# tvlearn/evo

Measured on AMD Instinct MI355X. Metric: E-step candidate-state evals/sec (NxS), full EM iteration, higher is better.
Workload: dtype f64; 1 GPU; ES3C D=256 H=512 S=200 N=100k f64 (north-star shape); algo=es3c, N_total=100000, N_rank0=100000, D=256, H=512, S=200, step=10 full EM iterations, world_size_rccl=1, ea=fit/randflip 10 parents x 1 child x 1 gen, states=p_init_Kn=1/H (init_states default), rng=device, mstep=device, parallelism=dp1

## Files before the change

### evo_amd/csrc/evo_amd.hip

```cpp
#include "../../include/evo_amd.h"

#include <dlfcn.h>
#include <math.h>
#include <stdarg.h>
#include <stdio.h>
#include <stdlib.h>
#include <string.h>

#include <atomic>
#include <chrono>
#include <memory>
#include <string>
#include <type_traits>
#include <vector>

#include "common.hpp"
#include "gemm_f64.hpp"
#include "kernels_bsc.hpp"
#include "kernels_common.hpp"
#include "kernels_evolve.hpp"
#include "kernels_mstep.hpp"
#include "kernels_sssc.hpp"
#include "kernels_sssc_quad.hpp"
#include "kernels_fused.hpp"
// ... 1906 lines not shown
  double expect = lv.scale * c->res_cnt[src] * ((tag == 0) ? 1.0 : 1.0 + (double)c->Cmax / (double)c->S);
  if (tag != 0 && level == 0) expect = (double)total;
  unsigned want = (unsigned)(2.0 * expect / per_block) + 4;
  return want < g ? want : g;
}

static bool use_k8_kernel(const evoamd_ctx *c, const LevelHints &lv) {
  const int tag = lv.known_tag;
  if (c->k8_mode >= 0) return c->k8_mode != 0;
  if (!c->need_known || tag == 2) return true;
  const double expect = c->res_cnt[tag == 0 ? 1 : 0] * (tag == 0 ? 1.0 : (double)c->Cmax / (double)c->S) +
                        (tag == 0 ? 0.0 : c->res_cnt[1]);
  return expect > 8192.0;
}

static bool few_dense_states(const evoamd_ctx *c, const LevelHints &lv) {
  const int tag = lv.known_tag;
  if (!c->need_known || tag == 2) return false;
  const double expect = lv.scale * (tag == 0 ? c->res_cnt[1] : c->res_cnt[1] + c->res_cnt[0] * (double)c->Cmax / (double)c->S);
  return expect <= 1024.0;
}

static bool few_above4(const evoamd_ctx *c, const LevelHints &lv) {
  if (!c->merge_small || !c->need_known || lv.known_tag == 2) return false;
  const double expect = lv.scale * c->res_cnt[1] * (1.0 + 4.0 * (double)c->Cmax / (double)std::max(1, c->S));
  return expect <= 256.0;
}

static int zero_lists(evoamd_ctx *c) {
  if (!c->lists_clean) {
    if (c->pending_skip)
      check_lists_kernel<<<1, 256, 0, c->stream>>>(c->list_n, 4 * LIST_SHARDS, c->pending_skip, c->err);
    else
      HIP_TRY(hipMemsetAsync(c->list_n, 0, 4 * LIST_SHARDS * sizeof(int), c->stream));
  }
  on_lists_claimed(c);
  return 0;
}

static int skip_mask(const bool need[3]) { return (need[0] ? 0 : 1) | (need[1] ? 0 : 2) | (need[2] ? 0 : 4); }

static bool census_mode(const evoamd_ctx *c) {
  return c->model == EVOAMD_MODEL_SSSC && c->clist && c->clist_n && c->ovf_rec && c->use_digest && c->dig && !c->mask_infr;
}

static int ensure_census(evoamd_ctx *c) {
  if (c->census_gen == c->kn_gen) return 0;
  const i64 total = c->N * (i64)c->S;
  if (!c->clist_clean) check_lists_kernel<<<1, 256, 0, c->stream>>>(c->clist_n, 4 * LIST_SHARDS, c->census_skip, c->err);
  on_census_claimed(c);
  unsigned grid = cdiv(total, CENSUS_T * CENSUS_PPT);
  if (grid > (unsigned)(8 * c->n_cu)) grid = (unsigned)(8 * c->n_cu);
  SpanGuard g(c, KID_MISC);
  census_kernel<<<grid, CENSUS_T, 0, c->stream>>>(c->dig, total, c->clist, (i64)c->clist_words(), c->clist_n, (int)list_cap(total), c->err);
  HIP_TRY(hipGetLastError());
  DBG_SYNC(c, "census");
  if (c->debug_poison_list) {
    c->debug_poison_list = 0;
    const int bad[1] = {0x7FFFFFF0}, one[1] = {1};
    HIP_TRY(hipMemcpyAsync(c->clist, bad, sizeof(int), hipMemcpyHostToDevice, c->stream));
    HIP_TRY(hipMemcpyAsync(c->clist_n, one, sizeof(int), hipMemcpyHostToDevice, c->stream));
    HIP_TRY(hipStreamSynchronize(c->stream));
    on_census_poisoned(c);
    return 0;
  }
  made_census(c);
  return 0;
}

static unsigned quad_grid(const evoamd_ctx *c, const LevelHints &lv, int level, i64 total, unsigned cap) {
  return level_grid(c, lv, level, total * 4, cap, 64);
}

static unsigned pb_clamp(const PairBins &pb, unsigned grid) {
  return pb.ent && grid > (unsigned)pb.nwg ? (unsigned)pb.nwg : grid;
}
#define PB_GRID_CHECK(pb, grid) \
  REQUIRE(!(pb).ent || (i64)(grid) <= (i64)(pb).nwg, "pair bins: producer grid exceeds the regions per bin (pb.nwg)")

template <class F>
static void with_hw(int hw, F &&f) {
  switch (hw) {
    case 1: f(std::integral_constant<int, 1>{}); break;
    case 2: f(std::integral_constant<int, 2>{}); break;
    case 4: f(std::integral_constant<int, 4>{}); break;
    case 8: f(std::integral_constant<int, 8>{}); break;
    case 16: f(std::integral_constant<int, 16>{}); break;
    default: f(std::integral_constant<int, 0>{}); break;
  }
}

template <typename F>
static void with_spl(int S, F &&f) {
  if (S <= 64) f(std::integral_constant<int, 1>{});
  else if (S <= 128) f(std::integral_constant<int, 2>{});
  else if (S <= 256) f(std::integral_constant<int, 4>{});
  else if (S <= 512) f(std::integral_constant<int, 8>{});
  else f(std::integral_constant<int, 16>{});
}
template <typename F>
static void with_cpl(int Cmax, F &&f) {
  if (Cmax <= 64) f(std::integral_constant<int, 1>{});
  else f(std::integral_constant<int, 4>{});
}

struct Es3cLists {
  ListOut o1, o2, o3;
  ListIn i1, i2, i3;
  ListIn cA, cB, cC;
  ListIn empty;
  ListOut none_out;
  ListIn none_in;
};

static Es3cLists es3c_lists(const evoamd_ctx *c, int cap) {
  Es3cLists ls = {};
  ls.o1 = {c->list1, c->list_n + 0 * LIST_SHARDS, cap};
  ls.o2 = {c->list2, c->list_n + 1 * LIST_SHARDS, cap};
  ls.o3 = {c->list3, c->list_n + 2 * LIST_SHARDS, cap};
  ls.i1 = {ls.o1.items, ls.o1.counts, cap};
  ls.i2 = {ls.o2.items, ls.o2.counts, cap};
  ls.i3 = {ls.o3.items, ls.o3.counts, cap};
  if (c->clist && c->clist_n) {
    ls.cA = {c->clist, c->clist_n, cap};
    ls.cB = {c->clist + c->clist_words(), c->clist_n + LIST_SHARDS, cap};
    ls.cC = {c->clist + 2 * c->clist_words(), c->clist_n + 2 * LIST_SHARDS, cap};
    ls.empty = {c->clist, c->clist_n + 3 * LIST_SHARDS, 0};
  }
  return ls;
}

template <int MODE, int TAG>
static int census_wavefront_levels(evoamd_ctx *c, const SsscArgs &a, const Es3cLists &ls, const bool need[3], bool few4,
                                   const LevelHints &lv, i64 total) {
  if (few4) {
    sssc_big_kernel<MODE, TAG><<<std::max(64u, level_grid(c, lv, 1, total * 256, 1024, 1)), 64, big_lds(SSSC_KCAP), c->stream>>>(
        a, need[1] ? ls.cB : ls.empty, ls.none_out, SSSC_KCAP, need[2] ? ls.cC : ls.empty, ls.i3);
    return 4;
  }
  sssc_big_kernel<MODE, TAG><<<std::max(256u, level_grid(c, lv, 2, total * 256, 8192, 1)), 64, big_lds(16), c->stream>>>(
      a, need[2] ? ls.cC : ls.empty, ls.o2, 16, ls.i3);
  if (!need[2]) return 4;
  sssc_big_kernel<MODE, TAG><<<level_grid(c, lv, 2, total * 256, 1024, 1), 64, big_lds(SSSC_KCAP), c->stream>>>(
      a, ls.i2, ls.none_out, SSSC_KCAP);
  return 2 | 4;
}

#define MAIN_LPJ_LDS_MAX (48 * 1024)

static size_t main_lpj_lds(int C, int H) {
  return ((size_t)(1024 / C + 2) * H + (H <= 512 ? (size_t)4 * H : 0)) * sizeof(double);
}

enum LpjRoute {
  LPJ_MASKED,
  LPJ_CENSUS,
  LPJ_CHAINS,
  LPJ_ROUND2
};
enum LpjMain {
  LPJ_MAIN_NONE,
  LPJ_MAIN_CENSUS,
  LPJ_MAIN_STAGED,
  LPJ_MAIN_UNSTAGED,
  LPJ_MAIN_SMALL
};

struct LpjPlan {
  LpjRoute route;
  LevelHints lv;
  int kid_main;
  i64 total;
  int cap;
  Es3cLists ls;
  bool need[3];
  bool any;
  LpjMain main;
  int rows_cap, stage_dg;
  size_t lds;
  unsigned grid;
  bool few4;
  bool k8;
  bool few_dense;
};

static void lpj_plan(const evoamd_ctx *c, const SsscArgs &a, int tag, const LevelHints &lv, int kid_main, LpjPlan &p) {
  p = LpjPlan{};
  p.lv = lv;
  p.kid_main = kid_main;
  p.total = a.N * (i64)a.C;
  p.cap = (int)list_cap(p.total);
  p.ls = es3c_lists(c, p.cap);
  levels_for(c, lv, p.need);
  p.any = p.need[0] || p.need[1] || p.need[2];
  const bool tables = !a.shared && (a.H % 2) == 0;
  const bool staged = tables && main_lpj_lds(a.C, a.H) <= MAIN_LPJ_LDS_MAX;
  if (a.mask)
    p.route = LPJ_MASKED;
  else if (tag == 0 && a.states == c->states && census_mode(c) && staged)
    p.route = LPJ_CENSUS;
  else
    p.route = c->census_opt ? LPJ_CHAINS : LPJ_ROUND2;
  p.stage_dg = a.H <= 512;
  p.grid = cdiv(p.total, 1024);
  if (staged) {
    p.main = p.route == LPJ_CENSUS ? (lv.levels_only ? LPJ_MAIN_NONE : LPJ_MAIN_CENSUS) : LPJ_MAIN_STAGED;
    p.rows_cap = 1024 / a.C + 2;
    p.lds = main_lpj_lds(a.C, a.H);
  } else if (tables && a.dig && c->main_unstaged) {
    p.main = LPJ_MAIN_UNSTAGED;
    p.lds = (p.stage_dg ? (size_t)4 * a.H : 0) * sizeof(double);
  } else {
    p.main = LPJ_MAIN_SMALL;
    p.grid = cdiv(p.total, 512);
  }
  p.few4 = p.route != LPJ_ROUND2 && few_above4(c, lv);
  p.k8 = p.route == LPJ_ROUND2 && use_k8_kernel(c, lv);
  p.few_dense = p.route == LPJ_ROUND2 && few_dense_states(c, lv);
}

static int lpj_sssc_masked(evoamd_ctx *c, const SsscArgs &a, const LpjPlan &p) {
  SpanGuard g(c, p.kid_main);
  const int gridm = (int)std::min<i64>(p.total, 65536);
  sssc_big_kernel<0><<<gridm, 64, big_lds(8), c->stream>>>(a, p.ls.none_in, p.ls.o3, 8);
  sssc_big_kernel<0><<<1024, 64, big_lds(SSSC_KCAP), c->stream>>>(a, p.ls.i3, p.ls.none_out, SSSC_KCAP);
  HIP_TRY(hipGetLastError());
  return 0;
}

template <int TAG>
static int lpj_sssc_main(evoamd_ctx *c, const SsscArgs &a, const LpjPlan &p) {
  if (p.main == LPJ_MAIN_NONE) return 0;
  SpanGuard g(c, p.kid_main);
  if (p.main == LPJ_MAIN_SMALL)
    sssc_small_kernel<2, 0, TAG, 512><<<p.grid, 512, 0, c->stream>>>(a, p.ls.none_in, p.ls.o1, PairBins{});
  else
    with_hw(a.HW, [&](auto hw) {
      constexpr int HWT = decltype(hw)::value;
      if (p.main == LPJ_MAIN_CENSUS)
        sssc_main_lpj_kernel<TAG, 512, HWT, 2, false><<<p.grid, 512, p.lds, c->stream>>>(a, p.ls.none_out, p.rows_cap, p.stage_dg);
      else if (p.main == LPJ_MAIN_STAGED)
        sssc_main_lpj_kernel<TAG, 512, HWT, 2><<<p.grid, 512, p.lds, c->stream>>>(a, p.ls.o1, p.rows_cap, p.stage_dg);
      else
        sssc_main_lpj_kernel<TAG, 512, HWT, 2, true, false><<<p.grid, 512, p.lds, c->stream>>>(a, p.ls.o1, 0, p.stage_dg);
    });
  HIP_TRY(hipGetLastError());
  DBG_SYNC(c, p.main == LPJ_MAIN_CENSUS ? "sssc lpj main (census)" : "sssc lpj main");
  return 0;
}

template <int TAG>
static int lpj_sssc_census_levels(evoamd_ctx *c, const SsscArgs &a, const LpjPlan &p, int &served) {
  const Es3cLists &ls = p.ls;
  SpanGuard g(c, KID_LPJ_OVF);
  if (p.need[0]) {
    SpanGuard gl(c, KID_LPJ_K34);
    sssc_quad_kernel<1, 0, TAG><<<quad_grid(c, p.lv, 0, p.total, 2048), 256, 0, c->stream>>>(a, ls.cA, ls.none_out, ls.o3, PairBins{}, nullptr);
  }
  DBG_SYNC(c, "sssc lpj quad level 3..4");
  if (p.need[1] && !p.few4) {
    SpanGuard gl(c, KID_LPJ_K58);
    sssc_quad_kernel<2, 0, TAG><<<quad_grid(c, p.lv, 1, p.total, 2048), 256, 0, c->stream>>>(a, ls.cB, ls.none_out, ls.o3, PairBins{}, nullptr);
  }
  DBG_SYNC(c, "sssc lpj quad level 5..8");
  SpanGuard gl(c, KID_LPJ_K9P);
  served = census_wavefront_levels<0, TAG>(c, a, ls, p.need, p.few4, p.lv, p.total);
  HIP_TRY(hipGetLastError());
  DBG_SYNC(c, p.few4 ? "sssc lpj census levels (merged)" : "sssc lpj census levels");
  return 0;
}

template <int TAG>
static int lpj_sssc_chain_levels(evoamd_ctx *c, const SsscArgs &a, const LpjPlan &p, int &served) {
  const Es3cLists &ls = p.ls;
  SpanGuard g(c, KID_LPJ_OVF);
  if (p.need[0])
    sssc_quad_kernel<1, 0, TAG><<<quad_grid(c, p.lv, 0, p.total, 2048), 256, 0, c->stream>>>(a, ls.i1, ls.o2, ls.o3, PairBins{}, nullptr);
  DBG_SYNC(c, "sssc lpj chain 3..4");
  if (p.few4) {
    sssc_big_kernel<0, TAG><<<std::max(64u, level_grid(c, p.lv, 1, p.total * 256, 1024, 1)), 64, big_lds(SSSC_KCAP), c->stream>>>(
        a, ls.i2, ls.none_out, SSSC_KCAP, ls.i3);
    served = 2 | 4;
  } else {
    if (p.need[1])
      sssc_quad_kernel<2, 0, TAG><<<quad_grid(c, p.lv, 1, p.total, 2048), 256, 0, c->stream>>>(a, ls.i2, ls.o3, ls.o3, PairBins{}, nullptr);
    DBG_SYNC(c, "sssc lpj chain 5..8");
    sssc_big_kernel<0, TAG><<<level_grid(c, p.lv, 2, p.total * 256, 1024, 1), 64, big_lds(SSSC_KCAP), c->stream>>>(
        a, ls.i3, ls.none_out, SSSC_KCAP);
    served = 4;
  }
  HIP_TRY(hipGetLastError());
  DBG_SYNC(c, p.few4 ? "sssc lpj chain wavefront level (merged)" : "sssc lpj chain wavefront level");
  return 0;
}

template <int TAG>
static int lpj_sssc_round2_levels(evoamd_ctx *c, const SsscArgs &a, const LpjPlan &p, int &served) {
  const Es3cLists &ls = p.ls;
  SpanGuard g(c, KID_LPJ_OVF);
  if (p.need[0])
    sssc_small_kernel<4, 0, TAG, 256><<<level_grid(c, p.lv, 0, p.total, 1024, 256), 256, 0, c->stream>>>(a, ls.i1, ls.o2, PairBins{}, ls.o3);
  DBG_SYNC(c, "sssc lpj K=4 level");
  bool merged23 = false;
  if (p.k8) {
    if (p.need[1])
      sssc_small_kernel<8, 0, TAG, 256><<<level_grid(c, p.lv, 1, p.total, 256, 256), 256, 0, c->stream>>>(a, ls.i2, ls.o3, PairBins{}, ls.o3);
  } else if (p.need[1] && p.few_dense) {
    sssc_big_kernel<0, TAG><<<level_grid(c, p.lv, 1, p.total * 256, 1024, 1), 64, big_lds(SSSC_KCAP), c->stream>>>(
        a, ls.i2, ls.none_out, SSSC_KCAP, ls.i3);
    merged23 = true;
  } else if (p.need[1]) {
    sssc_big_kernel<0, TAG><<<level_grid(c, p.lv, 1, p.total * 256, 4096, 1), 64, big_lds(8), c->stream>>>(a, ls.i2, ls.o3, 8);
  }
  DBG_SYNC(c, "sssc lpj K=8 level");
  if ((p.need[2] || c->sing_screen) && !merged23)
    sssc_big_kernel<0, TAG><<<level_grid(c, p.lv, 2, p.total * 256, 1024, 1), 64, big_lds(SSSC_KCAP), c->stream>>>(
        a, ls.i3, ls.none_out, SSSC_KCAP);
  served = (merged23 || p.need[2] || c->sing_screen) ? 4 : 0;
  HIP_TRY(hipGetLastError());
  DBG_SYNC(c, "sssc lpj wavefront level");
  return 0;
}

template <int TAG>
static int launch_sssc_lpj(evoamd_ctx *c, const SsscArgs &a, int kid_main, const LevelHints &lv) {
  TRY(zero_lists(c));
  LpjPlan p;
  lpj_plan(c, a, TAG, lv, kid_main, p);
  if (p.route == LPJ_MASKED) return lpj_sssc_masked(c, a, p);
  if (p.route == LPJ_CENSUS) TRY(ensure_census(c));
  TRY(lpj_sssc_main<TAG>(c, a, p));
  int served = 0;
  if (p.any)
    TRY(p.route == LPJ_CENSUS   ? lpj_sssc_census_levels<TAG>(c, a, p, served)
        : p.route == LPJ_CHAINS ? lpj_sssc_chain_levels<TAG>(c, a, p, served)
                                : lpj_sssc_round2_levels<TAG>(c, a, p, served));
  on_levels_skipped(c, p.route == LPJ_CENSUS, skip_mask(p.need), served, p.any);
  return 0;
}

static int launch_lpj(evoamd_ctx *c, const Batch &b, const LevelHints &lv) {
  if (c->model == EVOAMD_MODEL_BSC) return launch_bsc_lpj(c, b);
  SsscArgs a = sssc_args(c, b);
  if (b.tag == 0) return launch_sssc_lpj<0>(c, a, b.kid, lv);
  if (b.tag == 1) return launch_sssc_lpj<1>(c, a, b.kid, lv);
  return launch_sssc_lpj<2>(c, a, b.kid, lv);
}

static int check_err(evoamd_ctx *c) {
  int *e = c->h_err;
  HIP_TRY(hipMemcpyAsync(e, c->err, 4 * sizeof(int), hipMemcpyDeviceToHost, c->stream));
  HIP_TRY(hipStreamSynchronize(c->stream));
  if (e[0]) {
    HIP_TRY(hipMemsetAsync(c->err, 0, sizeof(int), c->stream));
    if (e[0] & 4) return fail(EVOAMD_E_INVALID, "internal: an ES3C overflow level was skipped although its list was not empty");
    if (e[0] & EVO_ERR_LIST_FULL) return fail(EVOAMD_E_INVALID, "internal: an ES3C overflow list was full, states were dropped");
    if (e[0] & EVO_ERR_BAD_ENTRY) return fail(EVOAMD_E_INVALID, "internal: an ES3C list entry or latent index read back from LDS was out of range");
    if (e[0] & 1) return fail(EVOAMD_E_KLIMIT, "ES3C: a state has more than %d active latents", SSSC_KCAP);
    return fail(EVOAMD_E_SINGULAR, "ES3C: exactly singular k x k system (the reference takes pinv here)");
  }
  return 0;
}

static int lpj_resident_launch(evoamd_ctx *c, double *out, const LevelHints &lv) {
  TRY(ensure_B(c));
  on_lpj_overwritten(c);
  if (c->S_perm) {
    allzero_lpj_kernel<<<cdiv(c->N, 256), 256, 0, c->stream>>>(c->yy, c->N, c->dpar, c->model == EVOAMD_MODEL_SSSC,
                                                               out, c->L, c->flags + 2 * c->N, c->err);
    HIP_TRY(hipGetLastError());
  }
  Batch b = {c->states, nullptr, c->Y, c->Bm, c->yy, c->N, c->S, 0, out, c->L, c->S_perm, c->flags, KID_LPJ_RES, 0};
  b.mask = c->mask_infr;
  SpanGuard pass(c, KID_LPJ_PASS);
  return launch_lpj(c, b, lv);
}

static int estep_resident_pass(evoamd_ctx *c) {
  if (c->prefetch_gen == c->gen) {
    drop_prefetch(c);
    std::swap(c->lpj, c->lpj_alt);
    return 0;
  }
  return lpj_resident_launch(c, c->lpj, batch_hints(c, 0));
}

static int estep_check_ready(const evoamd_ctx *c) {
  REQUIRE(c && c->configured && c->have_data && c->have_params, "configure, upload_data and set_params first");
  return 0;
}
static int estep_check_parents(const evoamd_ctx *c, int n_parents) {
  REQUIRE(n_parents >= 1 && n_parents <= c->S && n_parents <= 64, "n_parents must be in [1, min(S, 64)]");
  return 0;
}
static int estep_check_randflip(const evoamd_ctx *c, int n_parents, int n_children) {
  TRY(estep_check_ready(c));
  TRY(estep_check_parents(c, n_parents));
  REQUIRE(n_children >= 1 && n_children <= EV_MAX_CHILDREN && n_children <= c->H, "n_children must be in [1, min(8, H)]");
  REQUIRE(n_parents * n_children <= c->Cmax, "n_parents * n_children exceeds the configured Cmax");
  return 0;
// ... 2733 lines not shown
```

### evo_amd/csrc/kernels_sssc.hpp

```cpp
#pragma once
#include "common.hpp"
#include "kernels_mstep.hpp"
#include "pair_bins.hpp"

struct __attribute__((aligned(64))) PairEntry {
  double g01;
  double L;
  double l00, l01, l10, l11;
  double pad[2];
};
__device__ __forceinline__ bool pair_singular_L(double L) { return L == __builtin_inf(); }
__device__ __forceinline__ bool pair_singular_lam(double l00) { return !(fabs(l00) <= 1.7976931348623157e308); }

struct __attribute__((aligned(16))) OvfRec {
  unsigned short idx[8];
  double qn;
  double pad;
  double z[8];
};
static_assert(sizeof(OvfRec) == 96, "OvfRec is six 16-byte loads");

#define CS_SLICES 16
struct SsscArgs {
  const u64 *states;
// ... 593 lines not shown
      base = __shfl(base, leader, 64);
      if (over[p]) buf[base + __popcll(mask & ((1ull << lane) - 1ull))] = value[p];
    }
  }
  lds_barrier();
  if (threadIdx.x == 0) {
    const int n = ctl[0];
    ctl[1] = n ? atomicAdd(&lo.counts[shard], n) : 0;
  }
}
template <int BS>
__device__ __forceinline__ void append_begin(const ListOut &lo, int shard, int value, bool over, int *buf, int *ctl) {
  const int v[1] = {value};
  const bool o[1] = {over};
  append_begin<BS, 1>(lo, shard, v, o, buf, ctl);
}
template <int BS>
__device__ __forceinline__ void append_end(const ListOut &lo, int shard, const int *buf, const int *ctl, int *err = nullptr) {
  lds_barrier();
  const int n = ctl[0], start = ctl[1];
  if (n == 0) return;
  if (start < 0 || start + n > lo.cap) {
    if (err && threadIdx.x == 0) atomicOr(err, EVO_ERR_LIST_FULL);
    return;
  }
  const i64 dst = (i64)shard * lo.cap + start;
  for (int i = threadIdx.x; i < n; i += BS) lo.items[dst + i] = buf[i];
}

__device__ __forceinline__ double sssc_k2_value(const int k, const int idx0, const int idx1, const double4 *D1t, const double *Bn,
                                                const PairEntry &pe, const double yyn, const double s, int *err) {
#pragma clang fp contract(off)
  double4 d0 = make_double4(0.0, 0.0, 0.0, 0.0), d1 = make_double4(0.0, 0.0, 0.0, 0.0);
  double b0 = 0.0, b1 = 0.0, g01 = 0.0, L = 0.0, l00 = 0.0, l01 = 0.0, l10 = 0.0, l11 = 0.0;
  if (k >= 1) {
    d0 = D1t[idx0];
    b0 = Bn[idx0];
    L = d0.y;
    l00 = d0.w;
  }
  if (k == 2) {
    d1 = D1t[idx1];
    b1 = Bn[idx1];
    g01 = pe.g01;
    L = pe.L;
    l00 = pe.l00;
    l01 = pe.l01;
    l10 = pe.l10;
    l11 = pe.l11;
    if (pair_singular_L(pe.L) && pair_singular_lam(pe.l00)) atomicOr(err, 2);
  }
  const double v0 = fma(-g01, d1.x, fma(-d0.z, d0.x, b0));
  const double v1 = fma(-d1.z, d1.x, fma(-g01, d0.x, b1));
  const double rr = fma(-d1.x, b1 + v1, fma(-d0.x, b0 + v0, yyn));
  const double t0 = fma(l01, v1, l00 * v0), t1 = fma(l11, v1, l10 * v0);
  const double quad = fma(v1, t1, v0 * t0);
  return fma(-0.5 * s, fma(-s, quad, rr), L);
}

template <int TAG, int BS, int HWT, int PPT, bool APPEND = true, bool STAGEB = true>
__global__ __launch_bounds__(BS) void sssc_main_lpj_kernel(SsscArgs a, ListOut lo, int rows_cap, int stage_dg) {
  a.s2inv = a.dpar[DP_S2INV];
  extern __shared__ double smem[];
  __shared__ int ovf_buf[BS * PPT];
  __shared__ int ovf_ctl[2];
  double *Bs = smem;
  double4 *DGs = (double4 *)(smem + (STAGEB ? (size_t)rows_cap * a.H : 0));
  const i64 total = a.N * (i64)a.C;
  const i64 t0 = (i64)blockIdx.x * (BS * PPT);
  const i64 n_first = t0 / a.C;
  i64 n_last = (t0 + BS * PPT - 1) / a.C;
  if (n_last > a.N - 1) n_last = a.N - 1;
  const int rows = (int)(n_last - n_first + 1);
  bool live[PPT], over[PPT];
  int nloc[PPT], c[PPT], ktot[PPT], idx0[PPT], idx1[PPT], tv[PPT];
  double yyn[PPT];
  const float rC = 1.0f / (float)a.C;
#pragma unroll
  for (int p = 0; p < PPT; p++) {
    const i64 t = t0 + threadIdx.x + (i64)p * BS;
    tv[p] = (int)t;
    live[p] = t < total;
    nloc[p] = c[p] = ktot[p] = idx0[p] = idx1[p] = 0;
    yyn[p] = 0.0;
    if (live[p]) {
      const int off = (int)(t - n_first * a.C);
      int r = (int)(((float)off + 0.5f) * rC);
      if (r * a.C > off) r--;
      if ((r + 1) * a.C <= off) r++;
      nloc[p] = r;
      c[p] = off - r * a.C;
      live[p] = !(a.counts && c[p] >= a.counts[n_first + r]);
    }
  }
  u64 dgv[PPT];
#pragma unroll
  for (int p = 0; p < PPT; p++) {
    dgv[p] = 0ull;
    if (a.dig) {
      const i64 tc = live[p] ? (n_first + nloc[p]) * (i64)a.C + c[p] : 0;
      dgv[p] = a.dig[tc];
    } else if (live[p]) {
      const i64 n = n_first + nloc[p];
      load_state_k2<HWT>(a.states + ((a.shared ? 0 : n * (i64)a.C) + c[p]) * a.HW, a.HW, ktot[p], idx0[p], idx1[p]);
    }
    yyn[p] = a.yy[live[p] ? n_first + nloc[p] : 0];
  }
  {
    if (STAGEB) {
      const double2 *src = (const double2 *)(a.Bm + n_first * a.H);
      double2 *dst = (double2 *)Bs;
      const int n2 = rows * a.H / 2;
      for (int i = threadIdx.x; i < n2; i += BS) dst[i] = src[i];
    }
    if (stage_dg)
      for (int i = threadIdx.x; i < a.H; i += BS) DGs[i] = a.D1[i];
  }
  PairEntry pe[PPT];
#pragma unroll
  for (int p = 0; p < PPT; p++) {
    if (a.dig && live[p]) {
      ktot[p] = dig_k(dgv[p]);
      idx0[p] = dig_idx(dgv[p], 0);
      idx1[p] = dig_idx(dgv[p], 1);
    }
    over[p] = live[p] && ktot[p] > 2;
    const bool pair = live[p] && ktot[p] == 2;
    pe[p] = a.PT[pair ? (i64)idx0[p] * a.H + idx1[p] : 0];
  }
  const int shard = (int)(blockIdx.x & (LIST_SHARDS - 1));
  if (APPEND)
    append_begin<BS, PPT>(lo, shard, tv, over, ovf_buf, ovf_ctl);
  else
    lds_barrier();
  const double4 *D1t = stage_dg ? DGs : a.D1;
  const double s = a.s2inv;
#pragma unroll
  for (int p = 0; p < PPT; p++) {
    if (live[p] && !over[p]) {
      const int k = ktot[p];
      const double *Bn = STAGEB ? Bs + (size_t)nloc[p] * a.H
                                : a.Bm + (n_first + nloc[p]) * (i64)a.H;
      const double val = sssc_k2_value(k, idx0[p], idx1[p], D1t, Bn, pe[p], yyn[p], s, a.err);
      unsigned fl = 0;
      const i64 n = n_first + nloc[p];
      a.lpj_out[n * a.ldo + a.col0 + c[p]] = clamp_lpj(val, fl);
      if (fl) {
        atomicOr(&a.flags[n], fl);
        atomicOr(&a.err[1], 1);
      }
    }
  }
  if (APPEND) append_end<BS>(lo, shard, ovf_buf, ovf_ctl, a.err);
}

template <int HWT, int W, bool CEN = false>
__global__ __launch_bounds__(64 * W, W == 4 ? 2 : 1) void sssc_stats_wave_kernel(SsscArgs a, ListOut lo, PairBins pb, int stage,
                                                                                const OvfRec *__restrict__ rec = nullptr,
                                                                                const int rec_kmax = 8) {
  a.s2inv = a.dpar[DP_S2INV];
  extern __shared__ double wrows[];
  __shared__ int bcnt[PB_MAX_BINS];
  constexpr int OVB = 64;
  __shared__ int obuf[W][2 * OVB];
  const int H = a.H, lane = lane_id(), wave = wave_id_uniform();
  double *rowS = wrows + (size_t)wave * 2 * H, *rowZ = rowS + H;
  double *accS = wrows + (size_t)W * 2 * H, *accZ = accS + H, *accD = accZ + H;
  double *rowB = accD + H + (size_t)wave * H;
  double4 *d1s = (double4 *)(accD + H + (size_t)W * H);
  const bool binned = pb.ent != nullptr;
  for (int i = threadIdx.x; i < 3 * H; i += 64 * W) accS[i] = 0.0;
  if (HWT > 0 || stage)
    for (int i = threadIdx.x; i < H; i += 64 * W) d1s[i] = a.D1[i];
  if (binned)
    for (int i = threadIdx.x; i < pb.nb; i += 64 * W) bcnt[i] = CEN ? pb.gcnt[(size_t)i * pb.nwg + blockIdx.x] : 0;
  __syncthreads();
  const int shard = (int)(blockIdx.x & (LIST_SHARDS - 1));
  const double s = a.s2inv;
  int ocnt = 0;
  auto flush_obuf = [&]() {
    int base = 0;
    if (lane == 0) base = atomicAdd(&lo.counts[shard], ocnt);
    base = __shfl(base, 0, 64);
    for (int i = lane; i < ocnt; i += 64) {
      const int pos = base + i;
      if (pos >= 0 && pos < lo.cap)
        lo.items[(i64)shard * lo.cap + pos] = obuf[wave][i];
      else
        atomicOr(a.err, EVO_ERR_LIST_FULL);
    }
    ocnt = 0;
    lds_wave_fence();
  };
  constexpr bool PF = HWT > 0;
  constexpr int HB = PF ? HWT : 1;
  struct Pre {
    double rmax, rsum, B[HB], l[4];
    u64 d[4];
  };
  auto issue = [&](i64 nn, Pre &p) {
    p.rmax = a.rowmax[nn];
    p.rsum = a.rowsum[nn];
    const double *Bnn = a.Bm + nn * H;
#pragma unroll
    for (int i = 0; i < HB; i++) {
      const int h = lane + 64 * i;
      p.B[i] = Bnn[h < H ? h : H - 1];
    }
    const double *lpn = a.lpj_in + nn * a.ldo + a.col0;
    const u64 *dgn = a.dig + nn * (i64)a.C;
#pragma unroll
    for (int u = 0; u < 4; u++) {
      const int c = 64 * u + lane, cc = c < a.C ? c : 0;
      p.d[u] = dgn[cc];
      p.l[u] = lpn[cc];
    }
  };
  const i64 n_first = (i64)blockIdx.x * W + wave, n_stride = (i64)gridDim.x * W;
  Pre cur = {};
  if (PF && n_first < a.N) issue(n_first, cur);
  for (i64 n = n_first; n < a.N; n += n_stride) {
    const i64 n_next = n + n_stride < a.N ? n + n_stride : n;
    for (int h = lane; h < 2 * H; h += 64) rowS[h] = 0.0;
    double rmax, rsum;
    const double *Bn = a.Bm + n * H;
    if (PF) {
      rmax = cur.rmax;
      rsum = cur.rsum + EVO_F64_TINY;
#pragma unroll
      for (int i = 0; i < HB; i++) {
        const int h = lane + 64 * i;
        if (h < H) rowB[h] = cur.B[i];
      }
      Bn = rowB;
    } else {
      rmax = a.rowmax[n];
      rsum = a.rowsum[n] + EVO_F64_TINY;
      if (stage) {
        for (int h = lane; h < H; h += 64) rowB[h] = Bn[h];
        Bn = rowB;
      }
    }
    const double4 *D1t = (PF || stage) ? d1s : a.D1;
    const double *lp = a.lpj_in + n * a.ldo + a.col0;
    lds_wave_fence();
    auto group = [&](const int c0, auto first_tag) {
      constexpr bool first = decltype(first_tag)::value;
      constexpr int RG = 4;
      bool live[RG];
      int k[RG], idx0[RG], idx1[RG];
      double l[RG];
#pragma unroll
      for (int u = 0; u < RG; u++) {
        const int c = c0 + 64 * u + lane;
        live[u] = c < a.C;
        k[u] = idx0[u] = idx1[u] = 0;
        l[u] = 0.0;
        if (first) {
          const u64 d = cur.d[u];
          k[u] = live[u] ? dig_k(d) : 0;
          idx0[u] = dig_idx(d, 0);
          idx1[u] = dig_idx(d, 1);
          l[u] = cur.l[u];
        } else {
          if (a.dig) {
            const u64 d = a.dig[n * (i64)a.C + (live[u] ? c : 0)];
            k[u] = live[u] ? dig_k(d) : 0;
            idx0[u] = dig_idx(d, 0);
            idx1[u] = dig_idx(d, 1);
          } else if (live[u]) {
            load_state_k2<0>(a.states + (n * (i64)a.C + c) * a.HW, a.HW, k[u], idx0[u], idx1[u]);
          }
          l[u] = lp[live[u] ? c : 0];
        }
      }
      bool over[RG];
      int n_over = 0, my_off[RG];
#pragma unroll
      for (int u = 0; u < RG; u++) {
        over[u] = live[u] && k[u] > 2;
        my_off[u] = 0;
        if (!CEN) {
          const u64 om = __ballot(over[u]);
          my_off[u] = n_over + __popcll(om & ((1ull << lane) - 1ull));
          n_over += __popcll(om);
        }
      }
      const bool o_direct = !CEN && n_over > OVB;
      int obase = 0;
      if (o_direct) {
        if (lane == 0) obase = atomicAdd(&lo.counts[shard], n_over);
        obase = __shfl(obase, 0, 64);
      }
      int ofirst = -1;
      bool omore = false;
      OvfRec orec = {};
      if (CEN) {
#pragma unroll
        for (int u = RG - 1; u >= 0; u--)
          if (over[u] && k[u] <= rec_kmax) {
            omore = ofirst >= 0;
            ofirst = u;
          }
      }
      bool act[RG], pair[RG];
      PairEntry pe[RG];
// ... 832 lines not shown
```

Before: 5.085 billion state evals/s.

## Add wave-per-datapoint census LPJ main kernel with register prefetch

Adds a new census-route main log-joint kernel that gives each wavefront one datapoint at a time. Lanes cover candidate states, the B row is staged in per-wave LDS, and the next datapoint's digests, yy and B row are prefetched into registers while the current one is evaluated. The grid is sized to the resident wavefront count, with a grid-stride loop over datapoints. It aims to replace the block-of-512 staged kernel and its block-wide row staging with finer-grained, latency-hiding work. The path is gated on HW, C <= 256 (at most four states per lane) and an LDS budget, and it adds template instantiations and more register pressure.

```diff
diff --git a/evo_amd/csrc/evo_amd.hip b/evo_amd/csrc/evo_amd.hip
--- a/evo_amd/csrc/evo_amd.hip
+++ b/evo_amd/csrc/evo_amd.hip
@@ -2082,6 +2082,14 @@
   return ((size_t)(1024 / C + 2) * H + (H <= 512 ? (size_t)4 * H : 0)) * sizeof(double);
 }
 
+#define LPJ_WAVE_W 4
+static size_t lpj_wave_lds(int H) { return (size_t)(LPJ_WAVE_W + 4) * H * sizeof(double); }
+static unsigned lpj_wave_grid(const evoamd_ctx *c, i64 N, int H) {
+  const i64 per_cu = std::min<i64>(16 / LPJ_WAVE_W, (i64)(160 * 1024) / (i64)lpj_wave_lds(H));
+  const i64 resident = (i64)c->n_cu * per_cu, wgs = cdiv(N, LPJ_WAVE_W);
+  return (unsigned)(wgs <= 4 * resident ? wgs : resident);
+}
+
 enum LpjRoute {
   LPJ_MASKED,
   LPJ_CENSUS,
@@ -2091,6 +2099,7 @@
 enum LpjMain {
   LPJ_MAIN_NONE,
   LPJ_MAIN_CENSUS,
+  LPJ_MAIN_WAVE,
   LPJ_MAIN_STAGED,
   LPJ_MAIN_UNSTAGED,
   LPJ_MAIN_SMALL
@@ -2137,6 +2146,12 @@
     p.main = p.route == LPJ_CENSUS ? (lv.levels_only ? LPJ_MAIN_NONE : LPJ_MAIN_CENSUS) : LPJ_MAIN_STAGED;
     p.rows_cap = 1024 / a.C + 2;
     p.lds = main_lpj_lds(a.C, a.H);
+    const bool hw_fixed = a.HW == 1 || a.HW == 2 || a.HW == 4 || a.HW == 8 || a.HW == 16;
+    if (p.main == LPJ_MAIN_CENSUS && a.dig && !a.counts && a.C <= 256 && hw_fixed && lpj_wave_lds(a.H) <= 64 * 1024) {
+      p.main = LPJ_MAIN_WAVE;
+      p.lds = lpj_wave_lds(a.H);
+      p.grid = lpj_wave_grid(c, a.N, a.H);
+    }
   } else if (tables && a.dig && c->main_unstaged) {
     p.main = LPJ_MAIN_UNSTAGED;
     p.lds = (p.stage_dg ? (size_t)4 * a.H : 0) * sizeof(double);
@@ -2167,7 +2182,12 @@
   else
     with_hw(a.HW, [&](auto hw) {
       constexpr int HWT = decltype(hw)::value;
-      if (p.main == LPJ_MAIN_CENSUS)
+      if (p.main == LPJ_MAIN_WAVE)
+        with_spl(a.C, [&](auto spl) {
+          constexpr int R = decltype(spl)::value <= 4 ? decltype(spl)::value : 4;
+          sssc_lpj_wave_kernel<(HWT > 0 ? HWT : 1), LPJ_WAVE_W, R><<<p.grid, 64 * LPJ_WAVE_W, p.lds, c->stream>>>(a);
+        });
+      else if (p.main == LPJ_MAIN_CENSUS)
         sssc_main_lpj_kernel<TAG, 512, HWT, 2, false><<<p.grid, 512, p.lds, c->stream>>>(a, p.ls.none_out, p.rows_cap, p.stage_dg);
       else if (p.main == LPJ_MAIN_STAGED)
         sssc_main_lpj_kernel<TAG, 512, HWT, 2><<<p.grid, 512, p.lds, c->stream>>>(a, p.ls.o1, p.rows_cap, p.stage_dg);
@@ -2175,7 +2195,7 @@
         sssc_main_lpj_kernel<TAG, 512, HWT, 2, true, false><<<p.grid, 512, p.lds, c->stream>>>(a, p.ls.o1, 0, p.stage_dg);
     });
   HIP_TRY(hipGetLastError());
-  DBG_SYNC(c, p.main == LPJ_MAIN_CENSUS ? "sssc lpj main (census)" : "sssc lpj main");
+  DBG_SYNC(c, p.main == LPJ_MAIN_WAVE ? "sssc lpj main (census, wave per datapoint)" : p.main == LPJ_MAIN_CENSUS ? "sssc lpj main (census)" : "sssc lpj main");
   return 0;
 }
 
diff --git a/evo_amd/csrc/kernels_sssc.hpp b/evo_amd/csrc/kernels_sssc.hpp
--- a/evo_amd/csrc/kernels_sssc.hpp
+++ b/evo_amd/csrc/kernels_sssc.hpp
@@ -769,6 +769,81 @@
     }
   }
   if (APPEND) append_end<BS>(lo, shard, ovf_buf, ovf_ctl, a.err);
+}
+
+template <int HWT, int W, int R>
+__global__ __launch_bounds__(64 * W) void sssc_lpj_wave_kernel(SsscArgs a) {
+  static_assert(HWT > 0, "one register per 64 latents of the B row");
+  a.s2inv = a.dpar[DP_S2INV];
+  extern __shared__ double lrows[];
+  const int H = a.H, lane = lane_id(), wave = wave_id_uniform();
+  double *rowB = lrows + (size_t)wave * H;
+  double4 *d1s = (double4 *)(lrows + (size_t)W * H);
+  const double s = a.s2inv;
+  struct Pre {
+    double yy, B[HWT];
+    u64 d[R];
+  };
+  const unsigned h_last = (unsigned)lane + 64u * (HWT - 1);
+  auto issue = [&](i64 nn, Pre &p) {
+    const u64 *dgn = a.dig + nn * (i64)a.C;
+#pragma unroll
+    for (int u = 0; u < R; u++) {
+      const int c = 64 * u + lane;
+      p.d[u] = dgn[c < a.C ? c : 0];
+    }
+    p.yy = a.yy[nn];
+    const double *Bnn = a.Bm + nn * H;
+#pragma unroll
+    for (int i = 0; i < HWT - 1; i++) p.B[i] = Bnn[(unsigned)lane + 64u * i];
+    p.B[HWT - 1] = Bnn[h_last < H ? h_last : H - 1];
+  };
+  const i64 n_first = (i64)blockIdx.x * W + wave, n_stride = (i64)gridDim.x * W;
+  Pre cur;
+  issue(n_first < a.N ? n_first : a.N - 1, cur);
+  for (int i = threadIdx.x; i < H; i += 64 * W) d1s[i] = a.D1[i];
+  __syncthreads();
+  for (i64 n = n_first; n < a.N; n += n_stride) {
+    const i64 n_next = n + n_stride < a.N ? n + n_stride : n;
+    bool live[R], pair[R];
+    int k[R], idx0[R], idx1[R];
+#pragma unroll
+    for (int u = 0; u < R; u++) {
+      const u64 d = cur.d[u];
+      live[u] = 64 * u + lane < a.C;
+      k[u] = live[u] ? dig_k(d) : 0;
+      idx0[u] = dig_idx(d, 0);
+      idx1[u] = dig_idx(d, 1);
+    }
+    PairEntry pe[R];
+#pragma unroll
+    for (int u = 0; u < R; u++) {
+      pair[u] = k[u] == 2;
+      pe[u] = a.PT[pair[u] ? (i64)idx0[u] * H + idx1[u] : 0];
+    }
+#pragma unroll
+    for (int i = 0; i < HWT - 1; i++) rowB[lane + 64 * i] = cur.B[i];
+    if (h_last < H) rowB[h_last] = cur.B[HWT - 1];
+    const double yyn = cur.yy;
+    __builtin_amdgcn_sched_barrier(0);
+    issue(n_next, cur);
+    __builtin_amdgcn_sched_barrier(0);
+    lds_wave_fence();
+    double *out = a.lpj_out + n * a.ldo + a.col0;
+#pragma unroll
+    for (int u = 0; u < R; u++) {
+      if (live[u] && k[u] <= 2) {
+        const double val = sssc_k2_value(k[u], idx0[u], idx1[u], d1s, rowB, pe[u], yyn, s, a.err);
+        unsigned fl = 0;
+        out[64 * u + lane] = clamp_lpj(val, fl);
+        if (fl) {
+          atomicOr(&a.flags[n], fl);
+          atomicOr(&a.err[1], 1);
+        }
+      }
+    }
+    lds_wave_fence();
+  }
 }
 
 template <int HWT, int W, bool CEN = false>
```

After: 5.126 billion state evals/s, median of 6. About the same (+0.8%).
